# AUBVRL/H-SLAM

Hardware: AMD Instinct MI355X
Metric: point-residuals/sec in windowed photometric BA (8 KF × 2k pts), 1→8 GPU (higher is better)
Workload: dtype f32; 1 GPU; C4 (BASELINE.json configs[3]): full windowed photometric BA incl. Schur complement, 8 KF x 2000 pts, 640x480, 4 pyramid levels, strong scaling over 1 GPU(s) (2000 pts on rank 0); GN step = solve+step+linearize+accumulate (fp32 residuals, fp64 stitch/solve); frames=8, points=2000, points_per_gpu=2000, point_residuals=13634, parallelism=point-shard x1, launcher=single process

## Files before the change

### h-slam_amd/csrc/hs_ba_kernels.hip

```cpp
#pragma clang fp contract(off)
#include <hip/hip_runtime.h>

#include <cfloat>
#include <type_traits>

#include "hs_kernels.h"
#include "hs_se3_dev.h"


namespace {

constexpr float SCALE_F = 50.0f, SCALE_C = 50.0f, SCALE_IDEPTH = 1.0f;
constexpr int Q_N = 17;

__device__ __forceinline__ float3 interp33p(const float* __restrict__ img3, float x, float y, int w) {
  int ix = (int)x, iy = (int)y;
  float dx = x - ix, dy = y - iy, dxdy = dx * dy;
  const float* bp = img3 + 3 * (ix + iy * w);
  const float* bq = bp + 3 * w;
  const float3 p00 = make_float3(bp[0], bp[1], bp[2]), p10 = make_float3(bp[3], bp[4], bp[5]);
  const float3 p01 = make_float3(bq[0], bq[1], bq[2]), p11 = make_float3(bq[3], bq[4], bq[5]);
  const float w11 = dxdy, w01 = dy - dxdy, w10 = dx - dxdy, w00 = 1 - dx - dy + dxdy;
  float3 r;
  r.x = w11 * p11.x + w01 * p01.x + w10 * p10.x + w00 * p00.x;
  r.y = w11 * p11.y + w01 * p01.y + w10 * p10.y + w00 * p00.y;
  r.z = w11 * p11.z + w01 * p01.z + w10 * p10.z + w00 * p00.z;
  return r;
}

template <int CTRL>
__device__ __forceinline__ double dpp_f64(double v) {
  const long long b = __double_as_longlong(v);
  const int lo = __builtin_amdgcn_update_dpp(0, (int)b, CTRL, 0xf, 0xf, false);
  const int hi = __builtin_amdgcn_update_dpp(0, (int)(b >> 32), CTRL, 0xf, 0xf, false);
  return __longlong_as_double(((long long)hi << 32) | (unsigned int)lo);
}

__device__ __forceinline__ float dpp_shr1(float v) {
  return __int_as_float(__builtin_amdgcn_update_dpp(0, __float_as_int(v), 0x111, 0xf, 0xf, false));
}
__device__ __forceinline__ float octet_fold(float x) {
  float s = 0.f + x;
#pragma unroll
  for (int j = 0; j < 7; j++) s = dpp_shr1(s) + x;
  return s;
}
__device__ __forceinline__ float readlane_f(float v, int lane) {
  return __int_as_float(__builtin_amdgcn_readlane(__float_as_int(v), lane));
}

__device__ __forceinline__ float point_step(int p, int h, int nF, unsigned m, const float* cstep, const float* Hcd,
                                            float bdSumF, float HdiF, const int8_t* res_order, const float* xAd,
                                            const float* JpJdF) {
  if (m == 0u) return 0.f;
  float b = bdSumF;
  float dot = 0.f;
  for (int c = 0; c < 4; c++) dot += cstep[c] * Hcd[p * 4 + c];
  b -= dot;
  for (int q = 0; q < 8; q++) {
    const int tt = res_order[p * 8 + q];
    if (tt < 0) break;
    if (!((m >> tt) & 1u)) continue;
    const float* xa = xAd + (h * nF + tt) * 8;
    const float* jp = JpJdF + (p * 8 + tt) * 8;
    float d = 0.f;
    for (int i = 0; i < 8; i++) d += xa[i] * jp[i];
    b -= d;
  }
  return -b * HdiF;
}

__device__ __forceinline__ void frame_pose_stage(const double sc[10], const hs::SE3& evalPT, double* o,
                                                 hs::SE3* PWo = nullptr, hs::SE3* PCo = nullptr) {
  const hs::SE3 PW = se3_mul_step(se3_exp_step(sc), evalPT);
  const hs::SE3 PC = PW.inverse();
  PW.toData(o);
  PC.toData(o + 7);
  o[14] = sc[6];
  o[15] = sc[7];
  if (PWo) *PWo = PW;
  if (PCo) *PCo = PC;
}

template <typename PC>
__device__ __forceinline__ void pair_precalc_stage(const double* oh, const double* ot, float exp_h, float exp_t,
                                                   double state_zero7_h, const float vsf[4], PC& pc) {
  double aff[2];
  hs::fromToVecExposure(exp_h, exp_t, oh[14], oh[15], ot[14], ot[15], aff);
  pc.aff[0] = (float)aff[0];
  pc.aff[1] = (float)aff[1];
  pc.b0 = (float)(state_zero7_h * hs::SCALE_B);
  const float K[9] = {vsf[0], 0, vsf[2], 0, vsf[1], vsf[3], 0, 0, 1};
  float Ki[9];
  hs::inv3f(K, Ki);
  hs::SE3 PWt, PCh;
  PWt.q = hs::Quat{ot[0], ot[1], ot[2], ot[3]};
  PWt.t[0] = ot[4]; PWt.t[1] = ot[5]; PWt.t[2] = ot[6];
  PCh.q = hs::Quat{oh[7], oh[8], oh[9], oh[10]};
  PCh.t[0] = oh[11]; PCh.t[1] = oh[12]; PCh.t[2] = oh[13];
  const hs::SE3 l2l = se3_mul_step(PWt, PCh);
  double R[9];
  l2l.rotationMatrix(R);
  float RT[9], tT[3];
#pragma unroll
  for (int i = 0; i < 9; i++) RT[i] = (float)R[i];
#pragma unroll
  for (int i = 0; i < 3; i++) tT[i] = (float)l2l.t[i];
  float KR[9], KRKi[9], Kt[3];
  hs::mm3f(K, RT, KR);
  hs::mm3f(KR, Ki, KRKi);
  hs::mv3f(K, tT, Kt);
#pragma unroll
  for (int i = 0; i < 9; i++) pc.KRKi[i] = KRKi[i];
#pragma unroll
  for (int i = 0; i < 3; i++) pc.Kt[i] = Kt[i];
}

}

namespace {

struct LinPt {
  float Jx[10], Jy[10];
  float S[Q_N];
  float jj;
  bool active;
  unsigned mask;
  float HdiF, bdSumF, Hcd[4];
  double eSum;
  float idep;
  float xk, yk;
  float xr10, yr10, xc10, yc10;
  float xr14, yr14, t014, t114;
  float br15;
  float hcr, hcc;
};

struct LinIn {
  float idep, idep0, pu, pv;
  int res;
  int st_raw;
  float oldE_raw, oldNewE_raw;
  float colorK, weightK;
  uint2 ro2;
  unsigned fm;
  float jpj, bds, hdi;
  float4 hcd;
  float priorF;
};
__device__ __forceinline__ void lin_load(const HsLinArgs& a, int p, int lane, LinIn& in) {
  const int t = lane >> 3, k = lane & 7, sl = p * 8 + t;
  in.idep = a.idepth[p];
  in.idep0 = a.idepth_zero[p];
  in.pu = a.u[p];
  in.pv = a.v[p];
  in.res = a.res_of_slot[sl];
// ... 347 lines not shown
    unsigned long long am = __ballot(k < nres && (tq & 7) == t) & actBits;
    am |= am >> 4;
    am |= am >> 2;
    am |= am >> 1;
    am &= 0x0101010101010101ull;
    const unsigned mask = (unsigned)((am * 0x0102040810204080ull) >> 56);
    const double eSum = __longlong_as_double(((long long)__builtin_amdgcn_readlane((int)(__double_as_longlong(eAcc) >> 32), 7) << 32) |
                                             (unsigned int)__builtin_amdgcn_readlane((int)__double_as_longlong(eAcc), 7));
    const float bd = readlane_f(qsum, 0), Hdd = readlane_f(qsum, 1);
    float Hcd[4];
#pragma unroll
    for (int c = 0; c < 4; c++) Hcd[c] = readlane_f(qsum, 2 + c);
    float HdiF = 0.f, bdSumF = 0.f;
    if (mask != 0u) {
      const float priorF = (kMarg && a.marg) ? in.priorF * a.margPriorFac : in.priorF;
      float Hh = (kMarg && a.marg) ? (0.f + Hdd) + priorF : Hdd + 0.f + priorF;
      if ((double)Hh < 1e-10) Hh = (float)1e-10;
      HdiF = (float)(1.0 / (double)Hh);
      bdSumF = (kMarg && a.marg) ? 0.f + bd : bd + 0.f;
      if (!(kMarg && a.marg)) bdSumF += priorF * (idep - idep0);
    }
    float4 hc4;
    if (kMarg && a.marg) hc4 = make_float4(0.f + Hcd[0], 0.f + Hcd[1], 0.f + Hcd[2], 0.f + Hcd[3]);
    else hc4 = make_float4(Hcd[0] + 0.f, Hcd[1] + 0.f, Hcd[2] + 0.f, Hcd[3] + 0.f);
    {
      const float qh = (kMarg && a.marg) ? 0.f + qsum : qsum + 0.f;
      o.hcr = __shfl(qh, 2 + ((lane >> 2) & 3));
      o.hcc = __shfl(qh, 2 + (lane & 3));
    }
    if (lane == 0) {
      a.p_actmask[p] = (uint8_t)mask;
      a.p_HdiF[p] = HdiF;
      a.p_bdSumF[p] = bdSumF;
      reinterpret_cast<float4*>(a.p_Hcd)[p] = hc4;
    }
    if (kFix) {
      float q0 = pc.KRKi[0] * pu + pc.KRKi[1] * pv + pc.KRKi[2] * 1.f;
      float q1 = pc.KRKi[3] * pu + pc.KRKi[4] * pv + pc.KRKi[5] * 1.f;
      float q2 = pc.KRKi[6] * pu + pc.KRKi[7] * pv + pc.KRKi[8] * 1.f;
      const float r0 = q0 + pc.Kt[0] * idep, r1 = q1 + pc.Kt[1] * idep, r2 = q2 + pc.Kt[2] * idep;
      const float dx = q0 / q2 - r0 / r2, dy = q1 / q2 - r1 / r2;
      const float relBS = (float)(0.01 * (double)sqrtf(dx * dx + dy * dy));
      float mr = a.fix_relBL[p];
      int ng = a.fix_nGood[p];
      for (int qn = 0; qn < 8; qn++) {
        const int tt = res_slot(qn);
        if (tt < 0) break;
        if (!((actBits >> (tt * 8)) & 1ull)) continue;
        const float rb = readlane_f(relBS, tt * 8);
        if (rb > mr) mr = rb;
        ng++;
      }
      if (lane == 0) {
        a.fix_relBL[p] = mr;
        a.fix_nGood[p] = ng;
      }
    }
    o.mask = mask;
    o.HdiF = HdiF;
    o.bdSumF = bdSumF;
    o.Hcd[0] = hc4.x; o.Hcd[1] = hc4.y; o.Hcd[2] = hc4.z; o.Hcd[3] = hc4.w;
    o.eSum = eSum;
  }
  if (trc && threadIdx.x == 0 && o.eSum != -12345.0) trc[(size_t)blockIdx.x * 16 + 15] = wall_clock64();
#pragma unroll
  for (int i = 0; i < 10; i++) {
    o.Jx[i] = Jx[i];
    o.Jy[i] = Jy[i];
  }
#pragma unroll
  for (int i = 0; i < Q_N; i++) o.S[i] = S[i];
  o.active = active;
  o.idep = idep;
  {
    float xk = Jx[0], yk = Jy[0];
#pragma unroll
    for (int c = 1; c < 8; c++) {
      xk = k == c ? Jx[c] : xk;
      yk = k == c ? Jy[c] : yk;
    }
    o.xk = xk;
    o.yk = yk;
    o.xr10 = k == 2 ? Jx[9] : Jx[8];
    o.yr10 = k == 2 ? Jy[9] : Jy[8];
    o.xc10 = k == 0 ? Jx[8] : Jx[9];
    o.yc10 = k == 0 ? Jy[8] : Jy[9];
    const int kk = k < 3 ? k : k - 3;
    o.xr14 = k < 3 ? Jx[8] : Jx[9];
    o.yr14 = k < 3 ? Jy[8] : Jy[9];
    o.t014 = kk == 0 ? S[4] : (kk == 1 ? S[6] : S[12]);
    o.t114 = kk == 0 ? S[5] : (kk == 1 ? S[7] : S[13]);
    o.br15 = k == 0 ? S[8] : k == 1 ? S[9] : k == 2 ? S[14] : k == 3 ? S[10] : k == 4 ? S[15] : S[16];
  }
}

__host__ __device__ constexpr int dpair(int o1, int o2) { return o1 * 7 - (o1 * (o1 - 1)) / 2 + (o2 - o1); }

template <bool kExact>
struct LinAcc {
  static constexpr int ND = kExact ? HS_ND_EXACT : HS_ND_PROD;
  float T[HS_E_TOP];
  float D[ND];
  float E[5];
  float C;
  double e, sid, np;
};

template <bool kExact>
__device__ __forceinline__ void acc_point(LinAcc<kExact>& A, const LinPt& P, int h, int lane, float* ws) {
  if (P.active) {
    const float a_ = P.S[1], b_ = P.S[3], c_ = P.S[2];
    const float xk = P.xk, yk = P.yk;
    auto dat = [&](float xr, float yr, float xc, float yc) {
      return ((a_ * xc) * xr + (c_ * yc) * yr) + b_ * ((xc * yr) + (yc * xr));
    };
#pragma unroll
    for (int j = 0; j < 8; j++) A.T[j] += dat(P.Jx[j], P.Jy[j], xk, yk);
    A.T[8] += dat(xk, yk, P.Jx[8], P.Jy[8]);
    A.T[9] += dat(xk, yk, P.Jx[9], P.Jy[9]);
    A.T[10] += dat(P.xr10, P.yr10, P.xc10, P.yc10);
    A.T[11] += xk * P.S[4] + yk * P.S[5];
    A.T[12] += xk * P.S[6] + yk * P.S[7];
    A.T[13] += xk * P.S[12] + yk * P.S[13];
    A.T[14] += P.xr14 * P.t014 + P.yr14 * P.t114;
    A.T[15] += P.br15;
    const float wl = P.HdiF * P.jj;
#pragma unroll
    for (int c = 0; c < 4; c++) A.E[c] += wl * P.Hcd[c];
    A.E[4] += (P.HdiF * P.bdSumF) * P.jj;
  }
  {
    const int dr = lane >> 3, dc = lane & 7;
    float* jb = ws + LW_JJ;
    const int t = lane >> 3, k = lane & 7;
    if (t != h) jb[k * 8 + t - (t > h ? 1 : 0)] = P.jj;
    __builtin_amdgcn_wave_barrier();
    const float4 r0 = *reinterpret_cast<const float4*>(jb + dr * 8), r1 = *reinterpret_cast<const float4*>(jb + dr * 8 + 4);
    const float4 c0 = *reinterpret_cast<const float4*>(jb + dc * 8), c1 = *reinterpret_cast<const float4*>(jb + dc * 8 + 4);
    const float j1[7] = {r0.x, r0.y, r0.z, r0.w, r1.x, r1.y, r1.z};
    const float j2[7] = {c0.x, c0.y, c0.z, c0.w, c1.x, c1.y, c1.z};
#pragma unroll
    for (int o1 = 0; o1 < 7; o1++) {
      const float wl = P.HdiF * j1[o1];
#pragma unroll
      for (int o2 = kExact ? 0 : o1; o2 < 7; o2++) A.D[kExact ? o1 * 7 + o2 : dpair(o1, o2)] += wl * j2[o2];
    }
  }
  if (P.mask != 0u) A.C += lane < 16 ? (P.HdiF * P.hcr) * P.hcc : (P.bdSumF * P.HdiF) * P.hcc;
  A.e += P.eSum;
  A.sid += (double)fabsf(P.idep);
  A.np += 1.0;
}

template <bool kExact, bool kFix, bool kMarg = false, bool kProd = false>
__device__ __forceinline__ void lin_block(const HsLinArgs& a) {
  struct { long long* trace; } const T{kProd ? nullptr : a.trace};
  extern __shared__ float lin_stage[];
  if (a.brk && a.st->stop) return;
  const int tid = threadIdx.x, lane = tid & 63, wv = __builtin_amdgcn_readfirstlane(tid >> 6);
  const int b = blockIdx.x;
  int h = 0;
#pragma unroll
  for (int i = 1; i < HS_MAXF; i++) h += (i < a.nF && b >= a.blk_begin[i]) ? 1 : 0;
  const int nb = a.blk_begin[h + 1] - a.blk_begin[h], q = b - a.blk_begin[h];
  const int hb = a.host_begin[h], nh = a.host_begin[h + 1] - hb;
  const int pb = hb + (int)((long long)nh * q / nb), pe = hb + (int)((long long)nh * (q + 1) / nb);
  HS_TRACE(T, 0);
  __shared__ LinConst K;
  {
    const int nF = a.nF;
    constexpr int PW = (int)(sizeof(HsPrecalc) / 4);
    static_assert(sizeof(HsPrecalc) % 4 == 0, "precalc staged as words");
    const int* src = reinterpret_cast<const int*>(a.pre + h * nF);
    int* dst = reinterpret_cast<int*>(K.pre);
    for (int i = tid; i < nF * PW; i += HS_LIN_NT) dst[i] = src[i];
    if (tid < nF) K.th[tid] = a.frameTH[tid];
    if ((kProd || a.fuse_step) && tid < nF * 8) {
      const int t = tid >> 3, c = tid & 7;
      const float* aH = a.adHostF + (h + nF * t) * 64;
      const float* aT = a.adTargetF + (h + nF * t) * 64;
      const double* lx = a.st->lastX;
      float s1 = 0.f, s2 = 0.f;
#pragma unroll
      for (int rr = 0; rr < 8; rr++) s1 += (float)lx[4 + 8 * h + rr] * aH[rr * 8 + c];
#pragma unroll
      for (int rr = 0; rr < 8; rr++) s2 += (float)lx[4 + 8 * t + rr] * aT[rr * 8 + c];
      K.xad[tid] = s1 + s2;
    }
    if (tid < 4) K.cs[tid] = a.st->cstep[tid];
    if (tid >= 128 && tid < 128 + HS_MAXF) K.slot[tid - 128] = hs_img_slot(a.img_slot, tid - 128);
    constexpr int CW = (int)(sizeof(HsCalib) / 4);
    static_assert(sizeof(HsCalib) % 4 == 0, "calib staged as words");
    if (tid >= 64 && tid < 64 + CW)
      reinterpret_cast<int*>(&K.cal)[tid - 64] = reinterpret_cast<const int*>(&a.st->dcal)[tid - 64];
  }
  LinAcc<kExact> A;
#pragma unroll
  for (int i = 0; i < HS_E_TOP; i++) A.T[i] = 0.f;
#pragma unroll
  for (int i = 0; i < LinAcc<kExact>::ND; i++) A.D[i] = 0.f;
#pragma unroll
  for (int i = 0; i < 5; i++) A.E[i] = 0.f;
  A.C = 0.f;
  A.e = A.sid = A.np = 0.0;
  float* ws = lin_stage + wv * hs_ne(kExact) * 64;
  LinIn cur;
  const bool work = wv < a.W && pb + wv < pe;
  if (work) lin_load(a, pb + wv, lane, cur);
  __syncthreads();
  HS_TRACE(T, 12);
  if (work && pb + wv + a.W >= pe) {
    LinPt P;
    lin_point<kFix, kMarg, kProd>(a, pb + wv, h, lane, cur, K, ws, P);
    if (a.accumulate) acc_point<kExact>(A, P, h, lane, ws);
  } else if (work) {
    for (int p = pb + wv; p < pe; p += a.W) {
      typedef const HsLinArgs __attribute__((address_space(4))) * KArgs;
      KArgs ap = (KArgs)__builtin_amdgcn_kernarg_segment_ptr();
      asm volatile("" : "+s"(ap));
      const HsLinArgs& al = *(const HsLinArgs*)ap;
      LinIn nxt;
      if (p + al.W < pe) lin_load(al, p + al.W, lane, nxt);
      else nxt = cur;
      LinPt P;
      lin_point<kFix, kMarg, kProd>(al, p, h, lane, cur, K, ws, P);
      if (al.accumulate) acc_point<kExact>(A, P, h, lane, ws);
      cur = nxt;
    }
  }
  HS_TRACE(T, 1);
  if (T.trace && lane == 0) T.trace[(size_t)blockIdx.x * 16 + 4 + wv] = wall_clock64();
  if (!a.accumulate) return;
  constexpr int NE = hs_ne(kExact);
  float* my = lin_stage + wv * NE * 64;
#pragma unroll
  for (int i = 0; i < HS_E_TOP; i++) my[i * 64 + lane] = A.T[i];
#pragma unroll
  for (int i = 0; i < LinAcc<kExact>::ND; i++) my[(HS_E_TOP + i) * 64 + lane] = A.D[i];
#pragma unroll
  for (int i = 0; i < 5; i++) my[(HS_E_TOP + LinAcc<kExact>::ND + i) * 64 + lane] = A.E[i];
  my[(NE - 1) * 64 + lane] = A.C;
  double* se = reinterpret_cast<double*>(lin_stage + HS_LIN_NW * NE * 64);
  if (lane == 0) {
    se[wv * 3 + 0] = A.e;
    se[wv * 3 + 1] = A.sid;
    se[wv * 3 + 2] = A.np;
  }
  __syncthreads();
  HS_TRACE(T, 3);
  static_assert((NE * 64) % 4 == 0, "partials staged as float4");
  float4* out4 = reinterpret_cast<float4*>(a.part + (size_t)b * NE * 64);
  const float4* st4 = reinterpret_cast<const float4*>(lin_stage);
  constexpr int NI = (NE * 16 + HS_LIN_NT - 1) / HS_LIN_NT;
  float4 v[NI][HS_LIN_NW];
#pragma unroll
  for (int k = 0; k < NI; k++)
#pragma unroll
    for (int w = 0; w < HS_LIN_NW; w++) v[k][w] = st4[w * NE * 16 + min(tid + k * HS_LIN_NT, NE * 16 - 1)];
#pragma unroll
  for (int k = 0; k < NI; k++) {
    const int i = tid + k * HS_LIN_NT;
    float4 s = v[k][0];
    if (a.W == HS_LIN_NW) {
#pragma unroll
      for (int w = 1; w < HS_LIN_NW; w++) {
        s.x += v[k][w].x;
        s.y += v[k][w].y;
        s.z += v[k][w].z;
        s.w += v[k][w].w;
      }
    } else {
#pragma unroll
      for (int w = 1; w < HS_LIN_NW; w++)
        if (w < a.W) {
          s.x += v[k][w].x;
          s.y += v[k][w].y;
          s.z += v[k][w].z;
          s.w += v[k][w].w;
        }
    }
    if (i < NE * 16) out4[i] = s;
  }
  if (tid < 3) {
    double s = se[tid];
    for (int w = 1; w < a.W; w++) s += se[w * 3 + tid];
    a.part_e[(size_t)b * 4 + tid] = s;
  }
  HS_TRACE(T, 2);
}
}

static_assert(std::is_trivially_copyable<HsLinArgs>::value && sizeof(HsLinArgs) <= 4096, "HsLinArgs by value in the kernarg segment");
__global__ __launch_bounds__(HS_LIN_NT) void hs_k_lin(HsLinArgs a) { lin_block<false, false, false, true>(a); }
__global__ __launch_bounds__(HS_LIN_NT) void hs_k_lin_gen(HsLinArgs a) { lin_block<false, false>(a); }
__global__ __launch_bounds__(HS_LIN_NT) void hs_k_lin_exact(HsLinArgs a) { lin_block<true, false>(a); }
__global__ __launch_bounds__(HS_LIN_NT) void hs_k_lin_fix(HsLinArgs a) { lin_block<false, true>(a); }
__global__ __launch_bounds__(HS_LIN_NT) void hs_k_lin_exact_fix(HsLinArgs a) { lin_block<true, true>(a); }
__global__ __launch_bounds__(HS_LIN_NT) void hs_k_lin_marg(HsLinArgs a) { lin_block<false, false, true>(a); }
__global__ __launch_bounds__(HS_LIN_NT) void hs_k_lin_exact_marg(HsLinArgs a) { lin_block<true, false, true>(a); }

namespace {
__device__ void red_energy_block(const HsRedArgs& a) {
  __shared__ double red[3][256];
  const int tid = threadIdx.x;
  if (tid < 256) {
    double s[3] = {0.0, 0.0, 0.0};
    const int per = (a.nblk + 255) / 256, b0 = tid * per, b1 = min(a.nblk, b0 + per);
    for (int b = b0; b < b1; b++)
#pragma unroll
      for (int k = 0; k < 3; k++) s[k] += a.part_e[(size_t)b * 4 + k];
#pragma unroll
    for (int k = 0; k < 3; k++) red[k][tid] = s[k];
  }
  __syncthreads();
  for (int o = 128; o > 0; o >>= 1) {
    if (tid < o)
#pragma unroll
      for (int k = 0; k < 3; k++) red[k][tid] += red[k][tid + o];
    __syncthreads();
  }
  if (tid < 3) a.sysE[tid] = red[tid][0];
}

__device__ void red_th_hist_block(const HsRedArgs& a, int j) {
  __shared__ unsigned int hh[HS_TH_BINS];
  const int tid = threadIdx.x, nt = blockDim.x;
  for (int i = tid; i < HS_TH_BINS; i += nt) hh[i] = 0u;
  __syncthreads();
  const int total = a.nranks * a.stride;
  const int per = (total + a.nhist - 1) / a.nhist, i0 = j * per, i1 = min(total, i0 + per);
  for (int i = i0 + tid; i < i1; i += nt) {
    const unsigned int v = __float_as_uint(a.cand[i]);
    if (v <= 0x7f800000u) atomicAdd(&hh[v >> 19], 1u);
  }
  __syncthreads();
  for (int i = tid; i < HS_TH_BINS; i += nt)
    if (hh[i]) atomicAdd(&a.th_hist[i], hh[i]);
}

__device__ __forceinline__ unsigned int block_incl_scan(unsigned int x, unsigned int* wsum, unsigned int& total) {
  const int tid = threadIdx.x, lane = tid & 63, wv = tid >> 6, nw = blockDim.x >> 6;
#pragma unroll
  for (int o = 1; o < 64; o <<= 1) {
    const unsigned int y = __shfl_up(x, o);
    if (lane >= o) x += y;
  }
  if (lane == 63) wsum[wv] = x;
  __syncthreads();
  unsigned int off = 0, tot = 0;
  for (int w = 0; w < nw; w++) {
    const unsigned int v = wsum[w];
    off += w < wv ? v : 0u;
    tot += v;
  }
  __syncthreads();
  total = tot;
  return x + off;
}

constexpr int TH_CAP = 24576;

// ... 135 lines not shown
      src = a.th_surv;
      srcn = gs;
    }
  }
  if (n == 0) {
    if (tid == 0) a.frameTH[a.newest] = 12 * 12 * 8;
    return;
  }
  if (!multi) {
    for (int i0 = 0; i0 < total; i0 += TH_U * nt) {
      unsigned int v[TH_U];
#pragma unroll
      for (int u = 0; u < TH_U; u++) {
        const int i = i0 + u * nt + tid;
        v[u] = i < total ? __float_as_uint(a.cand[i]) : 0xffffffffu;
      }
#pragma unroll
      for (int u = 0; u < TH_U; u++)
        if (v[u] <= 0x7f800000u && (v[u] >> 19) == b1) {
          atomicAdd(&hist2[(v[u] >> 9) & 1023u], 1u);
          const unsigned int pos = atomicAdd(&ctl[2], 1u);
          if (pos < (unsigned int)cap) buf[pos] = v[u];
        }
    }
    __syncthreads();
    ns = ctl[2];
    if (ns <= (unsigned int)cap) {
      src = buf;
      srcn = ns;
    }
  }
  unsigned int b2 = 0, tot2 = 0;
  hist_pick(hist2, 1024, false, -1.f, kk, wsum, ctl, b2, kk, tot2);
  const unsigned int p2 = (b1 << 10) | b2;
  if (src) {
    for (unsigned int i = tid; i < srcn; i += nt) {
      const unsigned int v = src[i];
      if ((v >> 9) == p2) atomicAdd(&hist3[v & 511u], 1u);
    }
  } else {
    for (int i0 = 0; i0 < total; i0 += TH_U * nt) {
      unsigned int v[TH_U];
#pragma unroll
      for (int u = 0; u < TH_U; u++) {
        const int i = i0 + u * nt + tid;
        v[u] = i < total ? __float_as_uint(a.cand[i]) : 0xffffffffu;
      }
#pragma unroll
      for (int u = 0; u < TH_U; u++)
        if (v[u] <= 0x7f800000u && (v[u] >> 9) == p2) atomicAdd(&hist3[v[u] & 511u], 1u);
    }
  }
  __syncthreads();
  unsigned int b3 = 0, k3 = 0, tot3 = 0;
  hist_pick(hist3, 512, false, -1.f, kk, wsum, ctl, b3, k3, tot3);
  if (tid == 0) {
    const float nth = sqrtf(__uint_as_float((p2 << 9) | b3));
    float th = nth * a.facMedian;
    th = 26.0f * a.constWeight + th * (1 - a.constWeight);
    th = th * th;
    th *= a.overallWeight * a.overallWeight;
    a.frameTH[a.newest] = th;
  }
}
__device__ __forceinline__ void red_energy_th_block(const HsRedArgs& a, unsigned int* sm) {
  th_select_block(a, sm, TH_CAP, false);
}

__device__ __forceinline__ int top_oct_index(int R, int C) {
  int e, k;
  if (C < 8) { e = R; k = C; }
  else if (C < 10) {
    if (R < 8) { e = C; k = R; }
    else { e = 10; k = (R == 8 && C == 8) ? 0 : (R == 8 ? 1 : 2); }
  } else if (R < 10) {
    const int col = C - 10;
    if (R < 8) { e = 11 + col; k = R; }
    else { e = 14; k = (R - 8) * 3 + col; }
  } else {
    e = 15;
    k = R == 10 ? C - 10 : (R == 11 ? 2 + C - 10 : 5);
  }
  return e * 8 + k;
}
__device__ __forceinline__ double top_oct(const double* oct, int R, int C) { return oct[top_oct_index(R, C)]; }
__device__ __forceinline__ int a88_index(int ln) {
  const int R = 4 + (ln >> 3), C = 4 + (ln & 7);
  return top_oct_index(min(R, C), max(R, C));
}

__device__ __forceinline__ double mm8(const double* L, const double* M, int r, int c) {
  double s0 = 0.0, s1 = 0.0;
#pragma unroll
  for (int l = 0; l < 8; l += 2) {
    s0 = __builtin_fma(L[r * 8 + l], M[l * 8 + c], s0);
    s1 = __builtin_fma(L[r * 8 + l + 1], M[(l + 1) * 8 + c], s1);
  }
  return s0 + s1;
}
__device__ __forceinline__ double mm8t(const double* L, const double* M, int r, int c) {
  double s0 = 0.0, s1 = 0.0;
#pragma unroll
  for (int l = 0; l < 8; l += 2) {
    s0 = __builtin_fma(L[r * 8 + l], M[c * 8 + l], s0);
    s1 = __builtin_fma(L[r * 8 + l + 1], M[c * 8 + l + 1], s1);
  }
  return s0 + s1;
}
__device__ __forceinline__ double sandwich8(const double* L, const double* M, const double* R, double* scr, int lane) {
  const int r = lane >> 3, c = lane & 7;
  scr[lane] = mm8(L, M, r, c);
  __builtin_amdgcn_fence(__ATOMIC_RELEASE, "wavefront");
  __builtin_amdgcn_wave_barrier();
  __builtin_amdgcn_fence(__ATOMIC_ACQUIRE, "wavefront");
  const double v = mm8t(scr, R, r, c);
  __builtin_amdgcn_wave_barrier();
  return v;
}

constexpr int ST_NT = HS_STITCH_NT, ST_NW = ST_NT / 64;
constexpr int ST_LDS = 12288 + ST_NW * 64;
static_assert(2 * ST_LDS >= 1600 + TH_CAP, "the threshold select's LDS lives in the stitch block's scratch");
}

__device__ __forceinline__ void red_host_chunk(const HsRedArgs& a, int h, int q) {
  const int NE64 = a.ne * 64;
  const int e = q * (int)blockDim.x + (int)threadIdx.x;
  const int b0 = a.blk_begin[h], b1 = a.blk_begin[h + 1];
  if (e < NE64) {
    double s = 0.0;
    if (b1 - b0 <= 32) {
      float v[32];
      const int bl = max(b1 - 1, 0);
#pragma unroll
      for (int u = 0; u < 32; u++) v[u] = a.part[(size_t)min(b0 + u, bl) * NE64 + e];
#pragma unroll
      for (int u = 0; u < 32; u++)
        if (b0 + u < b1) s += (double)v[u];
    } else {
      for (int bb = b0; bb < b1; bb += 64) {
        float v[64];
#pragma unroll
        for (int u = 0; u < 64; u++) v[u] = a.part[(size_t)min(bb + u, b1 - 1) * NE64 + e];
#pragma unroll
        for (int u = 0; u < 64; u++)
          if (bb + u < b1) s += (double)v[u];
      }
    }
    a.hostsum[(size_t)h * NE64 + e] = s;
  }
}

__global__ __launch_bounds__(256) void hs_k_reduce(HsRedArgs a) {
  if (a.stop && *a.stop) return;
  const int nred = a.nF * a.Q;
  const int b = blockIdx.x;
  if (a.hist_only) {
    red_th_hist_block(a, b);
    return;
  }
  HS_TRACE(a, 0);
  if (b == nred) { red_energy_block(a); HS_TRACE(a, 15); return; }
  if (b > nred) { red_th_hist_block(a, b - nred - 1); HS_TRACE(a, 15); return; }
  red_host_chunk(a, b / a.Q, b % a.Q);
  HS_TRACE(a, 15);
}

__global__ __launch_bounds__(HS_STITCH_NT) void hs_k_th_pass2(HsRedArgs a) {
  __shared__ unsigned int sm[1600 + TH_CAP];
  if (a.stop && *a.stop) return;
  red_th_pass2_block(a, blockIdx.x, sm);
}

__global__ __launch_bounds__(HS_STITCH_NT) void hs_k_th_select(HsRedArgs a) {
  __shared__ unsigned int sm[1600 + TH_CAP];
  if (a.stop && *a.stop) return;
  red_energy_th_block(a, sm);
}

__device__ void stitch_diag_schur(const HsStitchArgs& a, const int f, double* lds) {
  const int nF = a.nF;
  const int tid = threadIdx.x, lane = tid & 63, wv = tid >> 6, r = lane >> 3, c = lane & 7;
  const int NE64 = a.ne * 64;
  const double* HSf = a.hostsum + (size_t)f * NE64;
  double* aHf = lds;
  double* Dq = aHf + 512;
  double* tS = Dq + 4096;
  double* scr = tS + 512;
  {
    constexpr int SU = (512 + 4096 + ST_NT - 1) / ST_NT;
    double v[SU];
    int dst[SU];
#pragma unroll
    for (int u = 0; u < SU; u++) {
      const int q = tid + ST_NT * u;
      const double* src = a.adHost;
      int d = -1;
      if (q < 512) {
        const int t = q >> 6, ln = q & 63;
        if (t < nF) {
          src = a.adHost + (size_t)(f + nF * t) * 64 + ln;
          d = q;
        }
      } else if (q < 512 + 4096) {
        const int qd = q - 512, x1 = qd >> 9, x2 = (qd >> 6) & 7, ln = qd & 63, rr = ln >> 3, cc = ln & 7;
        if (x1 < nF && x2 < nF && x1 != f && x2 != f) {
          const int o1 = x1 - (x1 > f ? 1 : 0), o2 = x2 - (x2 > f ? 1 : 0);
          int base, ls, cs;
          if (a.exact) { base = (HS_E_TOP + o1 * 7 + o2) * 64; ls = 8; cs = 1; }
          else if (o1 <= o2) { base = (HS_E_TOP + dpair(o1, o2)) * 64; ls = 8; cs = 1; }
          else { base = (HS_E_TOP + dpair(o2, o1)) * 64; ls = 1; cs = 8; }
          src = HSf + base + rr * ls + cc * cs;
          d = 512 + qd;
        }
      }
      v[u] = *src;
      dst[u] = d;
    }
#pragma unroll
    for (int u = 0; u < SU; u++)
      if (dst[u] >= 0) lds[dst[u]] = v[u];
  }
  __syncthreads();
  HS_TRACE(a, 1);
  double* sw = scr + wv * 64;
  for (int x = wv; x < nF - 1; x += ST_NW) {
    const int y = x + (x >= f ? 1 : 0);
    double v0 = 0.0, v1 = 0.0;
#pragma unroll
    for (int t2 = 0; t2 < HS_MAXF; t2++) {
      const double pv = mm8t(Dq + (y * 8 + t2) * 64, aHf + t2 * 64, r, c);
      const bool on = t2 < nF && t2 != f;
      if (t2 & 1) v1 = on ? v1 + pv : v1;
      else v0 = on ? v0 + pv : v0;
    }
    sw[lane] = v0 + v1;
    __builtin_amdgcn_fence(__ATOMIC_RELEASE, "wavefront");
    __builtin_amdgcn_wave_barrier();
    __builtin_amdgcn_fence(__ATOMIC_ACQUIRE, "wavefront");
    tS[y * 64 + lane] = mm8(aHf + y * 64, sw, r, c);
    __builtin_amdgcn_wave_barrier();
  }
  __syncthreads();
  HS_TRACE(a, 2);
  if (tid < 64) {
    double vS[HS_MAXF];
#pragma unroll
    for (int i = 0; i < HS_MAXF; i++) vS[i] = tS[i * 64 + lane];
    double hf = 0.0;
#pragma unroll
    for (int t1 = 0; t1 < HS_MAXF; t1++) hf = (t1 < nF && t1 != f) ? hf + vS[t1] : hf;
    if (a.aux_out) a.aux_out[f * 64 + lane] = hf;
    if (a.aux_sep) a.aux_sep[f * 64 + lane] = hf;
  }
}

__device__ __forceinline__ void stitch_block(const HsStitchArgs& a, int j, double* lds) {
  const int nF = a.nF, n = 4 + 8 * nF, nn = n * n, SL = nn + n;
  const int tid = threadIdx.x, lane = tid & 63, wv = tid >> 6, r = lane >> 3, c = lane & 7;
  const int NE64 = a.ne * 64;
  const int ND = a.exact ? HS_ND_EXACT : HS_ND_PROD;
  const int oE = (HS_E_TOP + ND) * 64;
  const int nFB = nF * (nF + 1) / 2;
  HS_TRACE(a, 0);
  if (j < nF) {
    stitch_diag_schur(a, j, lds);
    HS_TRACE(a, 15);
    return;
  }
  j -= nF;
  if (j == nFB + nF + 1) {
    if (!a.red.skip_threshold) red_energy_th_block(a.red, reinterpret_cast<unsigned int*>(lds));
    HS_TRACE(a, 15);
    return;
  }
  if (j > nFB + nF + 1) {
    red_th_pass2_block(a.red, j - (nFB + nF + 2), reinterpret_cast<unsigned int*>(lds));
    return;
  }
  auto adH = [&](int h, int t) { return a.adHost + (size_t)(h + nF * t) * 64; };
  auto adT = [&](int h, int t) { return a.adTarget + (size_t)(h + nF * t) * 64; };
  auto HS = [&](int h) { return a.hostsum + (size_t)h * NE64; };
  auto Dat = [&](int h, int t1, int t2, int& base, int& ls, int& cs) {
    const int o1 = t1 - (t1 > h ? 1 : 0), o2 = t2 - (t2 > h ? 1 : 0);
    if (a.exact) { base = (HS_E_TOP + o1 * 7 + o2) * 64; ls = 8; cs = 1; }
    else if (o1 <= o2) { base = (HS_E_TOP + dpair(o1, o2)) * 64; ls = 8; cs = 1; }
    else { base = (HS_E_TOP + dpair(o2, o1)) * 64; ls = 1; cs = 8; }
  };
  double* out = a.out;
  double* sepA = a.sep;
  double* sepS = a.sep ? a.sep + SL : nullptr;
  auto put = [&](int R, int C, double ha, double hs, bool diag) {
    if (out) out[R * n + C] = diag ? ha * a.lambda1 - hs * a.sc : ha - hs * a.sc;
    if (sepA) {
      sepA[R * n + C] = ha;
      sepS[R * n + C] = hs;
    }
  };

  if (j < nFB) {
    int f = 0, g = 0;
    {
      int q = j;
      while (q >= nF - f) { q -= nF - f; f++; }
      g = f + q;
    }
// ... 1121 lines not shown
```

Before: 348.2 million point-residuals/s.

## Overlap linearize-kernel prologue loads with the stop check and assign staging roles per wave

Result: faster. 359.1 million point-residuals/s (median of 6 runs) (+3.1%).

```diff
diff --git a/h-slam_amd/csrc/hs_ba_kernels.hip b/h-slam_amd/csrc/hs_ba_kernels.hip
--- a/h-slam_amd/csrc/hs_ba_kernels.hip
+++ b/h-slam_amd/csrc/hs_ba_kernels.hip
@@ -2,6 +2,7 @@
 #include <hip/hip_runtime.h>
 
 #include <cfloat>
+#include <cstddef>
 #include <type_traits>
 
 #include "hs_kernels.h"
@@ -655,47 +656,109 @@
   A.np += 1.0;
 }
 
+__device__ __forceinline__ void lin_args_touch(const HsLinArgs& a) {
+  asm volatile("" ::"s"(a.st), "s"(a.nF), "s"(a.pre), "s"(a.frameTH), "s"(a.adHostF), "s"(a.adTargetF), "s"(a.W), "s"(a.brk));
+  asm volatile("" ::"s"(a.idepth), "s"(a.idepth_zero), "s"(a.u), "s"(a.v), "s"(a.res_of_slot), "s"(a.r_state),
+               "s"(a.r_energy), "s"(a.r_newEnergy), "s"(a.color), "s"(a.weight), "s"(a.res_order), "s"(a.p_actmask),
+               "s"(a.p_JpJdF), "s"(a.p_bdSumF), "s"(a.p_HdiF_prev), "s"(a.p_Hcd), "s"(a.priorF));
+}
+
 template <bool kExact, bool kFix, bool kMarg = false, bool kProd = false>
 __device__ __forceinline__ void lin_block(const HsLinArgs& a) {
   struct { long long* trace; } const T{kProd ? nullptr : a.trace};
   extern __shared__ float lin_stage[];
-  if (a.brk && a.st->stop) return;
+  lin_args_touch(a);
   const int tid = threadIdx.x, lane = tid & 63, wv = __builtin_amdgcn_readfirstlane(tid >> 6);
-  const int b = blockIdx.x;
+  const int b = blockIdx.x, nF = a.nF;
   int h = 0;
 #pragma unroll
-  for (int i = 1; i < HS_MAXF; i++) h += (i < a.nF && b >= a.blk_begin[i]) ? 1 : 0;
-  const int nb = a.blk_begin[h + 1] - a.blk_begin[h], q = b - a.blk_begin[h];
-  const int hb = a.host_begin[h], nh = a.host_begin[h + 1] - hb;
-  const int pb = hb + (int)((long long)nh * q / nb), pe = hb + (int)((long long)nh * (q + 1) / nb);
+  for (int i = 1; i < HS_MAXF; i++) h += (i < nF && b >= a.blk_begin[i]) ? 1 : 0;
+  int bb = a.blk_begin[0], be = a.blk_begin[1], hb = a.host_begin[0], he = a.host_begin[1];
+#pragma unroll
+  for (int i = 1; i < HS_MAXF; i++) {
+    bb = h == i ? a.blk_begin[i] : bb;
+    be = h == i ? a.blk_begin[i + 1] : be;
+    hb = h == i ? a.host_begin[i] : hb;
+    he = h == i ? a.host_begin[i + 1] : he;
+  }
+  const int nb = be - bb, q = b - bb, nh = he - hb;
   HS_TRACE(T, 0);
   __shared__ LinConst K;
-  {
-    const int nF = a.nF;
-    constexpr int PW = (int)(sizeof(HsPrecalc) / 4);
-    static_assert(sizeof(HsPrecalc) % 4 == 0, "precalc staged as words");
-    const int* src = reinterpret_cast<const int*>(a.pre + h * nF);
-    int* dst = reinterpret_cast<int*>(K.pre);
-    for (int i = tid; i < nF * PW; i += HS_LIN_NT) dst[i] = src[i];
-    if (tid < nF) K.th[tid] = a.frameTH[tid];
-    if ((kProd || a.fuse_step) && tid < nF * 8) {
-      const int t = tid >> 3, c = tid & 7;
-      const float* aH = a.adHostF + (h + nF * t) * 64;
-      const float* aT = a.adTargetF + (h + nF * t) * 64;
-      const double* lx = a.st->lastX;
-      float s1 = 0.f, s2 = 0.f;
-#pragma unroll
-      for (int rr = 0; rr < 8; rr++) s1 += (float)lx[4 + 8 * h + rr] * aH[rr * 8 + c];
-#pragma unroll
-      for (int rr = 0; rr < 8; rr++) s2 += (float)lx[4 + 8 * t + rr] * aT[rr * 8 + c];
-      K.xad[tid] = s1 + s2;
-    }
-    if (tid < 4) K.cs[tid] = a.st->cstep[tid];
-    if (tid >= 128 && tid < 128 + HS_MAXF) K.slot[tid - 128] = hs_img_slot(a.img_slot, tid - 128);
-    constexpr int CW = (int)(sizeof(HsCalib) / 4);
-    static_assert(sizeof(HsCalib) % 4 == 0, "calib staged as words");
-    if (tid >= 64 && tid < 64 + CW)
-      reinterpret_cast<int*>(&K.cal)[tid - 64] = reinterpret_cast<const int*>(&a.st->dcal)[tid - 64];
+  constexpr int PW = (int)(sizeof(HsPrecalc) / 4), CW = (int)(sizeof(HsCalib) / 4);
+  static_assert(sizeof(HsPrecalc) % 4 == 0 && sizeof(HsCalib) % 4 == 0, "precalc and calib staged as words");
+  static_assert(HS_LIN_NW == 8 && HS_MAXF * PW <= 4 * 64 && HS_MAXF * 8 <= 64 && CW <= 64 && HS_MAXF <= 8,
+                "the prologue's roles: one word per lane");
+  static_assert(offsetof(LinConst, pre) % 4 == 0 && offsetof(LinConst, th) % 4 == 0 &&
+                    offsetof(LinConst, cs) % 4 == 0 && offsetof(LinConst, slot) % 4 == 0,
+                "LinConst staged as words");
+  const bool fuse = kProd || a.fuse_step;
+  int vz;
+  asm volatile("v_mov_b32 %0, 0" : "=v"(vz));
+  typedef const int __attribute__((address_space(1))) * GInt;
+  const GInt stw = (GInt)(&a.st->stop + vz);
+  const int stopw = *stw;
+  const int pb = hb + (int)((long long)nh * q / nb), pe = hb + (int)((long long)nh * (q + 1) / nb);
+  LinIn cur;
+  const bool work = wv < a.W && pb + wv < pe;
+  lin_load(a, max(min(pb + wv, he - 1), 0), lane, cur);
+  GInt src = stw;
+  int dsti = 0;
+  bool sto = false;
+  if (wv >= 4) {
+    const int i = tid - 4 * 64;
+    src = (GInt)reinterpret_cast<const int*>(a.pre + h * nF) + min(i, nF * PW - 1);
+    dsti = (int)(offsetof(LinConst, pre) / 4) + i;
+    sto = i < nF * PW;
+  } else if (wv == 2) {
+    src = (GInt)reinterpret_cast<const int*>(&a.st->dcal) + min(lane, CW - 1);
+    dsti = (int)(offsetof(LinConst, cal) / 4) + lane;
+    sto = lane < CW;
+  } else if (wv == 3) {
+    const GInt ks = (GInt)reinterpret_cast<const int*>(
+        reinterpret_cast<const char*>((const void*)__builtin_amdgcn_kernarg_segment_ptr()) + offsetof(HsLinArgs, img_slot));
+    const int j = lane & 7;
+    src = lane < 8 ? (GInt)reinterpret_cast<const int*>(a.frameTH) + min(j, nF - 1)
+                   : lane < 16 ? (GInt)reinterpret_cast<const int*>(a.st->cstep) + (j & 3) : ks + j;
+    dsti = lane < 8 ? (int)(offsetof(LinConst, th) / 4) + j
+                    : lane < 16 ? (int)(offsetof(LinConst, cs) / 4) + (j & 3) : (int)(offsetof(LinConst, slot) / 4) + j;
+    sto = lane < 8 ? j < nF : lane < 16 ? j < 4 : lane < 16 + HS_MAXF;
+  }
+  int cw = *src;
+  typedef double d2 __attribute__((ext_vector_type(2), aligned(8)));
+  float xaH[8], xaT[8];
+  d2 xlH[4], xlT[4];
+  const bool xad = wv == 1 && fuse;
+  if (xad) {
+    const int t = min(lane >> 3, nF - 1), c = lane & 7;
+    const float* aH = a.adHostF + (h + nF * t) * 64 + c;
+    const float* aT = a.adTargetF + (h + nF * t) * 64 + c;
+    const d2* lH = reinterpret_cast<const d2*>(a.st->lastX + 4 + 8 * h + vz);
+    const d2* lT = reinterpret_cast<const d2*>(a.st->lastX + 4 + 8 * t);
+#pragma unroll
+    for (int rr = 0; rr < 8; rr++) {
+      xaH[rr] = aH[rr * 8];
+      xaT[rr] = aT[rr * 8];
+    }
+#pragma unroll
+    for (int rr = 0; rr < 4; rr++) {
+      xlH[rr] = lH[rr];
+      xlT[rr] = lT[rr];
+    }
+  }
+  asm volatile("" ::: "memory");
+  if (a.brk && __builtin_amdgcn_readfirstlane(stopw)) return;
+  asm volatile("" : "+v"(cw));
+  if (sto) reinterpret_cast<int*>(&K)[dsti] = cw;
+  if (xad) {
+    asm volatile("" : "+v"(xaH[0]), "+v"(xaH[1]), "+v"(xaH[2]), "+v"(xaH[3]), "+v"(xaH[4]), "+v"(xaH[5]), "+v"(xaH[6]), "+v"(xaH[7]),
+                      "+v"(xaT[0]), "+v"(xaT[1]), "+v"(xaT[2]), "+v"(xaT[3]), "+v"(xaT[4]), "+v"(xaT[5]), "+v"(xaT[6]), "+v"(xaT[7]));
+    asm volatile("" : "+v"(xlH[0]), "+v"(xlH[1]), "+v"(xlH[2]), "+v"(xlH[3]), "+v"(xlT[0]), "+v"(xlT[1]), "+v"(xlT[2]), "+v"(xlT[3]));
+    float s1 = 0.f, s2 = 0.f;
+#pragma unroll
+    for (int rr = 0; rr < 8; rr++) s1 += (float)xlH[rr >> 1][rr & 1] * xaH[rr];
+#pragma unroll
+    for (int rr = 0; rr < 8; rr++) s2 += (float)xlT[rr >> 1][rr & 1] * xaT[rr];
+    if (lane < nF * 8) K.xad[lane] = s1 + s2;
   }
   LinAcc<kExact> A;
 #pragma unroll
@@ -707,9 +770,6 @@
   A.C = 0.f;
   A.e = A.sid = A.np = 0.0;
   float* ws = lin_stage + wv * hs_ne(kExact) * 64;
-  LinIn cur;
-  const bool work = wv < a.W && pb + wv < pe;
-  if (work) lin_load(a, pb + wv, lane, cur);
   __syncthreads();
   HS_TRACE(T, 12);
   if (work && pb + wv + a.W >= pe) {
@@ -1151,6 +1211,8 @@
 }
 
 __global__ __launch_bounds__(256) void hs_k_reduce(HsRedArgs a) {
+  asm volatile("" ::"s"(a.stop), "s"(a.hist_only), "s"(a.nF), "s"(a.Q), "s"(a.ne), "s"(a.nblk), "s"(a.part),
+               "s"(a.hostsum), "s"(a.trace));
   if (a.stop && *a.stop) return;
   const int nred = a.nF * a.Q;
   const int b = blockIdx.x;
```
